# asonnino/hotstuff

Measured on NVIDIA H100. Metric: Ed25519 verifies/s, higher is better.
Workload: dtype u32

## Files before the change

hotstuff_b200/csrc/hs_engine.cu:

```cuda
#include <cuda_runtime.h>
#include <pthread.h>
#include <algorithm>
#include <array>
#include <atomic>
#include <chrono>
#include <condition_variable>
#include <cstdint>
#include <cstdio>
#include <cstdlib>
#include <cstring>
#include <deque>
#include <type_traits>
#include <initializer_list>
#include <list>
#include <memory>
#include <mutex>
#include <new>
#include <optional>
#include <random>
#include <string>
#include <string_view>
#include <system_error>
#include <thread>
#include <unordered_map>
#include <vector>

#include "../../include/hs_crypto.h"
#include "hs_args.h"
#include "hs_selftest_vectors.h"
#include "key_index.h"
#include "verify_core.cuh"

#define HS_THREADS 128
#define HS_FINISH_GROUP 16
#define HS_LEARN_MAX 8192u
#define HS_LEARN_PER_CALL 1024u
#define HS_CACHE_RESET_MIN_CALLS 64u

struct in_layout {
  const uint8_t *sig;
  size_t sig_stride;
  const uint8_t *pk;
  size_t pk_stride;
  const uint32_t *vidx;
  const uint8_t *msg;
  size_t msg_stride;
  const uint32_t *midx;
  const uint64_t *off;
  uint64_t fixed_len;
  int aos128;
};

__device__ __forceinline__ void load32(uint32_t (&w)[8], const uint8_t *p) {
  const uint32_t *s = reinterpret_cast<const uint32_t *>(p);
#pragma unroll
  for (int i = 0; i < 8; i++) w[i] = __ldg(s + i);
}
__device__ __forceinline__ void unpack8(uint32_t (&w)[8], uint4 lo, uint4 hi) {
  w[0] = lo.x; w[1] = lo.y; w[2] = lo.z; w[3] = lo.w;
  w[4] = hi.x; w[5] = hi.y; w[6] = hi.z; w[7] = hi.w;
}
__device__ __forceinline__ void store_digest32(uint32_t *dst, const uint32_t *h) {
  uint4 *d = reinterpret_cast<uint4 *>(dst);
  d[0] = make_uint4(h[0], h[1], h[2], h[3]);
  d[1] = make_uint4(h[4], h[5], h[6], h[7]);
}

template <class I, class Row>
__device__ __forceinline__ void warp_stage_rows128(uint4 (&q)[8], I n, I warp_first, Row row, uint4 *smem_warp, int lane) {
#pragma unroll
  for (int j = 0; j < 8; j++) {
    const int c = j * 32 + lane;
    const int rec = c >> 3, part = c & 7;
    const uint4 *src = row(rec);
    uint4 v = make_uint4(0, 0, 0, 0);
    if (warp_first + rec < n) v = __ldg(src + part);
    smem_warp[rec * 8 + (part ^ (rec & 7))] = v;
  }
  __syncwarp();
#pragma unroll
  for (int part = 0; part < 8; part++) q[part] = smem_warp[lane * 8 + (part ^ (lane & 7))];
}
__device__ __forceinline__ void warp_load_rec128(uint32_t (&sig_r)[8], uint32_t (&sig_s)[8], uint32_t (&pk)[8], uint32_t (&msg)[8],
                                                 const uint8_t *__restrict__ recs, size_t n, size_t warp_first, uint4 *smem_warp) {
  uint4 q[8];
  warp_stage_rows128(q, n, warp_first, [&](int r) { return reinterpret_cast<const uint4 *>(recs + (warp_first + r) * 128); }, smem_warp,
                     threadIdx.x & 31);
  __syncwarp();
  unpack8(sig_r, q[0], q[1]);
  unpack8(sig_s, q[2], q[3]);
  unpack8(pk, q[4], q[5]);
  unpack8(msg, q[6], q[7]);
}

struct key_table {
  const uint32_t *slots;
  uint32_t mask;
  const uint8_t *pks;
  uint32_t n_keys;
};
template <bool BOUNDED>
__device__ __forceinline__ uint32_t key_probe(const key_table &T, const uint32_t (&k)[8], uint32_t &pos) {
  uint32_t h = key_hash(k) & T.mask;
  for (uint32_t probe = 0; probe <= T.mask; probe++) {
    uint32_t idx = __ldg(T.slots + h);
    if (idx == HS_NO_KEY) break;
    if (!BOUNDED || idx < T.n_keys) {
      const uint32_t *cand = reinterpret_cast<const uint32_t *>(T.pks + (size_t)idx * 32);
      uint32_t diff = 0;
#pragma unroll
      for (int j = 0; j < 8; j++) diff |= __ldg(cand + j) ^ k[j];
      if (diff == 0) {
        pos = h;
        return idx;
      }
    }
    h = (h + 1) & T.mask;
  }
  return HS_NO_KEY;
}
__global__ void __launch_bounds__(256) k_key_lookup(in_layout L, size_t n, key_table T, uint32_t *__restrict__ out_vidx,
                                                    uint32_t *__restrict__ miss_list, uint32_t *__restrict__ miss_count) {
  const size_t i = (size_t)blockIdx.x * 256 + threadIdx.x;
  if (i >= n) return;
  uint32_t k[8];
  load32(k, L.pk + i * L.pk_stride);
  uint32_t pos;
  const uint32_t found = key_probe<false>(T, k, pos);
  out_vidx[i] = found;
  if (found == HS_NO_KEY) miss_list[atomicAdd(miss_count, 1u)] = (uint32_t)i;
}

__global__ void __launch_bounds__(256) k_gather_keys(in_layout L, size_t n, const uint32_t *__restrict__ miss_list,
                                                     const uint32_t *__restrict__ miss_count, uint32_t max_keys, uint8_t *__restrict__ out_keys,
                                                     uint32_t *__restrict__ out_n) {
  const size_t t = (size_t)blockIdx.x * 256 + threadIdx.x;
  const size_t avail = miss_count ? (size_t)*miss_count : n;
  const size_t take = avail < max_keys ? avail : max_keys;
  if (t == 0) *out_n = (uint32_t)take;
  if (t >= take) return;
  const size_t i = miss_count ? miss_list[t] : t;
  uint32_t k[8];
  load32(k, L.pk + i * L.pk_stride);
  uint32_t *dst = reinterpret_cast<uint32_t *>(out_keys + t * 32);
#pragma unroll
  for (int j = 0; j < 8; j++) dst[j] = k[j];
}

struct main_out {
  fe *xyz;
  uint8_t *meta;
  int side_pass;
};
struct committee_tables {
  const uint8_t *pks;
  const uint8_t *key_flags;
  uint32_t n_keys;
  const ge_niels *atables;
  size_t table_entries;
};

template <bool COMMITTEE>
#ifndef HS_MAIN_MINBLOCKS
#define HS_MAIN_MINBLOCKS 4
#endif
#ifndef HS_GENERIC_MINBLOCKS
#define HS_GENERIC_MINBLOCKS 3
#endif
__global__ void __launch_bounds__(HS_THREADS, COMMITTEE ? HS_MAIN_MINBLOCKS : HS_GENERIC_MINBLOCKS) k_verify_main(in_layout L, size_t n_arg, const uint32_t *__restrict__ n_ptr,
                                                             const uint32_t *__restrict__ index_list, const ge_niels *__restrict__ btable,
                                                             committee_tables C, main_out O, const comb_params cp) {
  __shared__ __align__(16) unsigned char smem_raw[HS_MAX_DIGITS * HS_THREADS * 4];
  static_assert(sizeof(smem_raw) >= (HS_THREADS / 32) * 256 * sizeof(uint4), "staging does not fit");
  uint4(*stage)[256] = reinterpret_cast<uint4(*)[256]>(smem_raw);
  int32_t *digits = reinterpret_cast<int32_t *>(smem_raw) + threadIdx.x;
  const size_t n = n_ptr ? (size_t)*n_ptr : n_arg;
  for (size_t base = (size_t)blockIdx.x * blockDim.x; base < n; base += (size_t)gridDim.x * blockDim.x) {
  const size_t t = base + threadIdx.x;
  const size_t warp_first = t & ~(size_t)31;
  const bool active = t < n;
  size_t i = active ? t : n - 1;
  uint32_t R[8], S[8], A[8], h[16];
  uint32_t v = 0;
  bool have_key = true;
  if (L.aos128 && !index_list) {
    uint32_t M[8];
    __syncthreads();
    warp_load_rec128(R, S, A, M, L.sig, n, warp_first, stage[threadIdx.x >> 5]);
    __syncthreads();
    if (COMMITTEE) {
      v = __ldg(L.vidx + i);
      have_key = v < C.n_keys;
      if (!have_key) v = 0;
      load32(A, C.pks + (size_t)v * 32);
    }
    sha512_ram32(h, R, A, M);
  } else {
    if (index_list) i = index_list[i];
    load32(R, L.sig + i * L.sig_stride);
    load32(S, L.sig + i * L.sig_stride + 32);
    if (COMMITTEE) {
      v = __ldg(L.vidx + i);
      have_key = v < C.n_keys;
      if (!have_key) v = 0;
      load32(A, C.pks + (size_t)v * 32);
    } else {
      load32(A, L.pk + i * L.pk_stride);
    }
    const uint8_t *m = L.off ? L.msg + L.off[i] : L.msg + (size_t)(L.midx ? __ldg(L.midx + i) : i) * L.msg_stride;
    const uint64_t len = L.off ? (L.off[i + 1] - L.off[i]) : L.fixed_len;
    if (len == 32 && ((reinterpret_cast<uintptr_t>(m) & 3u) == 0)) {
      uint32_t M[8];
      load32(M, m);
      sha512_ram32(h, R, A, M);
    } else {
      uint64_t pre[8];
#pragma unroll
      for (int j = 0; j < 4; j++) {
        pre[j] = be64_from_le32(R[2 * j], R[2 * j + 1]);
        pre[4 + j] = be64_from_le32(A[2 * j], A[2 * j + 1]);
      }
      sha512_prefix_msg(h, pre, 8, m, len);
    }
  }
  ge_ext acc;
  uint32_t meta;
  if (COMMITTEE) {
    meta = verify_committee_main(acc, R, S, h, btable, C.atables + (size_t)v * C.table_entries, have_key ? C.key_flags[v] : 0u, digits,
                                 HS_THREADS, cp);
    if (!have_key) {
      if (O.side_pass) continue;
      meta = 0;
    }
  } else {
    ge_cached tab[9];
    meta = verify_generic_main(acc, R, S, A, h, btable, tab, digits, HS_THREADS, cp);
  }
  if (!active) continue;
  if (!(meta & HS_META_PARSE_OK)) {
    fe_set0(acc.X);
    fe_set1(acc.Y);
    fe_set1(acc.Z);
  }
  uint4 *dst = reinterpret_cast<uint4 *>(O.xyz + i * 3);
  dst[0] = make_uint4(acc.X.v[0], acc.X.v[1], acc.X.v[2], acc.X.v[3]);
  dst[1] = make_uint4(acc.X.v[4], acc.X.v[5], acc.X.v[6], acc.X.v[7]);
  dst[2] = make_uint4(acc.Y.v[0], acc.Y.v[1], acc.Y.v[2], acc.Y.v[3]);
  dst[3] = make_uint4(acc.Y.v[4], acc.Y.v[5], acc.Y.v[6], acc.Y.v[7]);
  dst[4] = make_uint4(acc.Z.v[0], acc.Z.v[1], acc.Z.v[2], acc.Z.v[3]);
  dst[5] = make_uint4(acc.Z.v[4], acc.Z.v[5], acc.Z.v[6], acc.Z.v[7]);
  O.meta[i] = (uint8_t)meta;
  }
}

struct small_rec {
  uint8_t sig[64];
  uint8_t msg[32];
  uint32_t vidx;
  uint32_t req;
  uint32_t req_n;
  uint32_t pad[5];
};
static_assert(sizeof(small_rec) == 128, "small_rec is 128 bytes");
#define HS_SMALL_MAX 64
__device__ __forceinline__ void fe_shfl_down(fe &r, const fe &a, int delta) {
#pragma unroll
  for (int i = 0; i < 8; i++) r.v[i] = __shfl_down_sync(0xffffffffu, a.v[i], delta);
}

#define HS_SIG_WAYS 4
struct sig_entry {
  uint32_t w[32];
  uint32_t seq;
  uint32_t flags;
  uint32_t pad[2];
};
static_assert(sizeof(sig_entry) == 144, "sig_entry is 144 bytes");
struct sig_bucket {
  sig_entry e[HS_SIG_WAYS];
  uint32_t rr;
  uint32_t pad[3];
};
#define HS_SIG_CTRS 4
struct sig_cache_dev {
  sig_bucket *b;
  const uint64_t *key;
  uint32_t bmask;
  uint32_t *ctr;
  uint32_t *hctr;
};
#define HS_SIG_HIT 0x100u

__device__ __forceinline__ uint32_t ld_acquire_gpu(const uint32_t *p) {
  uint32_t v;
  asm volatile("ld.acquire.gpu.global.u32 %0, [%1];" : "=r"(v) : "l"(p) : "memory");
  return v;
}
__device__ __forceinline__ uint32_t ld_relaxed_gpu(const uint32_t *p) {
  uint32_t v;
  asm volatile("ld.relaxed.gpu.global.u32 %0, [%1];" : "=r"(v) : "l"(p) : "memory");
  return v;
}
__device__ __forceinline__ void st_relaxed_gpu(uint32_t *p, uint32_t v) {
  asm volatile("st.relaxed.gpu.global.u32 [%0], %1;" ::"l"(p), "r"(v) : "memory");
}
__device__ __forceinline__ uint64_t sig_mix(uint32_t w, uint64_t k) {
  uint64_t z = ((uint64_t)w << 32) ^ k;
  z = (z ^ (z >> 30)) * 0xbf58476d1ce4e5b9ull;
  z = (z ^ (z >> 27)) * 0x94d049bb133111ebull;
  return z ^ (z >> 31);
}
__device__ __forceinline__ uint32_t sig_bucket_of(const sig_cache_dev &sc, uint64_t h) { return (uint32_t)(h >> 32) & sc.bmask; }
__device__ __forceinline__ uint32_t pick8(const uint32_t (&a)[8], int i) {
  uint32_t r = a[0];
#pragma unroll
  for (int j = 1; j < 8; j++)
    if (i == j) r = a[j];
  return r;
}
__device__ __forceinline__ uint32_t sig_probe_warp(const sig_cache_dev &sc, uint32_t w, int lane, uint32_t &bucket) {
  uint64_t h = sig_mix(w, __ldg(sc.key + lane));
#pragma unroll
  for (int d = 16; d; d >>= 1) h += __shfl_xor_sync(0xffffffffu, h, d);
  bucket = sig_bucket_of(sc, h);
  const sig_entry *x = sc.b[bucket].e;
  uint32_t s0[HS_SIG_WAYS], m[HS_SIG_WAYS], f[HS_SIG_WAYS];
#pragma unroll
  for (int e = 0; e < HS_SIG_WAYS; e++) s0[e] = ld_acquire_gpu(&x[e].seq);
#pragma unroll
  for (int e = 0; e < HS_SIG_WAYS; e++) {
    m[e] = ld_relaxed_gpu(x[e].w + lane);
    f[e] = ld_relaxed_gpu(&x[e].flags);
  }
  __threadfence();
#pragma unroll
  for (int e = 0; e < HS_SIG_WAYS; e++) {
    const uint32_t s1 = ld_relaxed_gpu(&x[e].seq), s_lane0 = __shfl_sync(0xffffffffu, s0[e], 0), fl = __shfl_sync(0xffffffffu, f[e], 0);
    const bool ok = s0[e] != 0 && !(s0[e] & 1u) && s1 == s0[e] && s0[e] == s_lane0 && m[e] == w;
    if (__all_sync(0xffffffffu, ok)) return fl | HS_SIG_HIT;
  }
  return 0;
}
template <class W>
__device__ __forceinline__ uint32_t sig_probe_thread(const sig_cache_dev &sc, W word, uint32_t &bucket) {
  uint64_t h = 0;
#pragma unroll
  for (int j = 0; j < 32; j++) h += sig_mix(word(j), __ldg(sc.key + j));
  bucket = sig_bucket_of(sc, h);
  const sig_entry *x = sc.b[bucket].e;
#pragma unroll 1
  for (int e = 0; e < HS_SIG_WAYS; e++) {
    const uint32_t s0 = ld_acquire_gpu(&x[e].seq);
    if (!s0 || (s0 & 1u) || ld_relaxed_gpu(x[e].w) != word(0)) continue;
    bool eq = true;
#pragma unroll
    for (int j = 1; j < 32; j++) eq &= ld_relaxed_gpu(x[e].w + j) == word(j);
    const uint32_t fl = ld_relaxed_gpu(&x[e].flags);
    __threadfence();
    if (eq && ld_relaxed_gpu(&x[e].seq) == s0) return fl | HS_SIG_HIT;
  }
  return 0;
}
template <class W>
__device__ __forceinline__ uint32_t sig_insert(const sig_cache_dev &sc, uint32_t bucket, W word, uint32_t flags) {
// ... 1364 lines not shown
    cp.na = sc_ndigits_rt(w);
    sc_bias_rt(cp.bias_a, w);
  } else {
    cp.wb = w;
    cp.nb = sc_ndigits_rt(w);
    sc_bias_rt(cp.bias_b, w);
  }
}

static int audit_fence(hs_ctx *c, cudaStream_t stream) {
  c->key_gen++;
  c->map_gen++;
  if (c->audit.done) HS_CUDA(c, cudaStreamWaitEvent(stream, c->audit.done, 0));
  return HS_OK;
}
static void cache_release(hs_ctx *c) {
  c->key_gen++;
  c->map_gen++;
  c->keys = {};
  c->n_keys = 0;
  c->h_pks.clear();
  c->h_index = {};
  c->h_key_live.clear();
  c->stage = {};
  c->key_capacity = 0;
}
static int cache_allocate(hs_ctx *c, cudaStream_t stream) {
  size_t free_b = 0, total_b = 0;
  HS_CUDA(c, cudaMemGetInfo(&free_b, &total_b));
  size_t lim = free_b / 2;
  if (c->table_budget && c->table_budget < lim) lim = c->table_budget;
  int wa = 8;
  for (int w : {14, 12, 10, 8}) {
    if (c->wa_forced && w != c->wa_forced && w != 8) continue;
    wa = w;
    if (c->cache_cap * comb_table_entries(w) * sizeof(ge_niels) <= lim) break;
  }
  if (c->cache_cap * comb_table_entries(wa) * sizeof(ge_niels) > lim || sc_ndigits_rt(wa) + c->cp.nb > HS_MAX_DIGITS) {
    c->cache_enabled = false;
    return HS_OK;
  }
  set_window(c->cp, true, wa);
  c->a_table_entries = comb_table_entries(wa);
  HS_CUDA(c, make_key_store(c->keys, c->cache_cap, key_index::capacity_for(c->cache_cap), wa, stream));
  c->key_gen++;
  c->map_gen++;
  c->h_index.reset(c->cache_cap);
  c->h_pks.clear();
  return HS_OK;
}
static int learn_process(hs_ctx *c, cudaStream_t stream) {
  if (!c->learn_pending) return HS_OK;
  if (cudaEventQuery(c->learn.ev) != cudaSuccess) return HS_OK;
  c->learn_pending = false;
  c->calls_since_reset++;
  if (!c->cache_enabled || c->explicit_committee) return HS_OK;
  if (c->cache_full) {
    if (c->learn_records >= 64 && (size_t)*c->learn.h_miss_total * 2 > c->learn_records && c->calls_since_reset >= HS_CACHE_RESET_MIN_CALLS) {
      c->calls_since_reset = 0;
      HS_TRY(audit_fence(c, stream));
      c->n_keys = 0;
      c->h_pks.clear();
      c->h_index.clear();
      HS_CUDA(c, cudaMemsetAsync(c->keys.slots, 0xff, c->h_index.slots.size() * 4, stream));
      c->cache_full = false;
    }
    return HS_OK;
  }
  const uint32_t got = *c->learn.h_n < HS_LEARN_MAX ? *c->learn.h_n : HS_LEARN_MAX;
  if (got == 0) return HS_OK;
  if (!c->keys.atables) {
    HS_TRY(cache_allocate(c, stream));
    if (!c->cache_enabled) return HS_OK;
  }
  const size_t old_n = c->n_keys;
  size_t n_new = 0;
  for (uint32_t t = 0; t < got && old_n + n_new < c->cache_cap && n_new < HS_LEARN_PER_CALL; t++) {
    const uint8_t *key = c->learn.h_keys + 32 * (size_t)t;
    c->h_pks.insert(c->h_pks.end(), key, key + 32);
    if (c->h_index.insert_absent(c->h_pks.data(), (uint32_t)(old_n + n_new))) n_new++;
    else c->h_pks.resize(32 * (old_n + n_new));
  }
  if (n_new == 0) return HS_OK;
  HS_TRY(audit_fence(c, stream));
  HS_CUDA(c, cudaMemcpyAsync(c->keys.pks + old_n * 32, c->h_pks.data() + old_n * 32, n_new * 32, cudaMemcpyHostToDevice, stream));
  HS_CUDA(c, cudaMemcpyAsync(c->keys.slots, c->h_index.slots.data(), c->h_index.slots.size() * 4, cudaMemcpyHostToDevice, stream));
  HS_TRY(launch_build(c, c->keys.pks + old_n * 32, nullptr, n_new, 1, c->cp.wa, c->cp.na, c->keys.atables + old_n * c->a_table_entries,
                      c->keys.key_flags + old_n, stream));
  HS_CUDA(c, cudaEventRecord(c->learn.ev_tables, stream));
  c->n_keys = old_n + n_new;
  if (c->n_keys >= c->cache_cap) c->cache_full = true;
  return HS_OK;
}
static int learn_collect(hs_ctx *c, const in_layout &L, size_t n, bool have_lookup, cudaStream_t stream) {
  if (!c->cache_enabled || c->explicit_committee || c->learn_pending || !L.pk) return HS_OK;
  if (!c->learn.keys) {
    learn_bufs B;
    HS_CUDA(c, alloc(B.keys, (size_t)HS_LEARN_MAX * 32));
    HS_CUDA(c, alloc(B.n, 4));
    HS_CUDA(c, alloc(B.h_keys, (size_t)HS_LEARN_MAX * 32));
    HS_CUDA(c, alloc(B.h_n, 4));
    HS_CUDA(c, alloc(B.h_miss_total, 4));
    HS_CUDA(c, create(B.ev));
    HS_CUDA(c, create(B.ev_tables));
    c->learn = std::move(B);
  }
  learn_bufs &B = c->learn;
  c->learn_records = n;
  if (c->cache_full) {
    if (!have_lookup) return HS_OK;
    HS_CUDA(c, cudaMemcpyAsync(B.h_miss_total, c->d_miss_count, 4, cudaMemcpyDeviceToHost, stream));
    HS_CUDA(c, cudaEventRecord(B.ev, stream));
    c->learn_pending = true;
    return HS_OK;
  }
  k_gather_keys<<<blocks_for(HS_LEARN_MAX, 256), 256, 0, stream>>>(L, n, have_lookup ? (const uint32_t *)c->miss.p.get() : nullptr,
                                                                     have_lookup ? c->d_miss_count.get() : nullptr, HS_LEARN_MAX, B.keys, B.n);
  c->launches++;
  HS_CUDA(c, cudaGetLastError());
  HS_CUDA(c, cudaMemcpyAsync(B.h_n, B.n, 4, cudaMemcpyDeviceToHost, stream));
  HS_CUDA(c, cudaMemcpyAsync(B.h_keys, B.keys, (size_t)HS_LEARN_MAX * 32, cudaMemcpyDeviceToHost, stream));
  HS_CUDA(c, cudaEventRecord(B.ev, stream));
  c->learn_pending = true;
  return HS_OK;
}

struct pass_scratch {
  fe *xyz;
  uint8_t *meta;
  uint32_t *vidx, *miss, *miss_count;
  cudaStream_t side;
  cudaEvent_t ev_side[2];
  const event_h *prof;
};
struct pass_tables {
  committee_tables C;
  key_table T;
  comb_params cp;
};
static pass_tables store_tables(const key_store &S, const key_index &index, size_t n_keys, size_t entries, const comb_params &cp) {
  return pass_tables{{S.pks, S.key_flags, (uint32_t)n_keys, S.atables, entries}, {S.slots, index.mask, S.pks, (uint32_t)n_keys}, cp};
}
static pass_tables ctx_tables(const hs_ctx *c) { return store_tables(c->keys, c->h_index, c->n_keys, c->a_table_entries, c->cp); }
struct share_pass {
  sig_cache_dev sc;
  uint32_t *list;
  uint8_t *fl;
  uint32_t *h_ctr;
};
static int wait_key_cache_build(hs_ctx *c, cudaStream_t stream) {
  if (c->learn.ev_tables && !c->explicit_committee) HS_CUDA(c, cudaStreamWaitEvent(stream, c->learn.ev_tables, 0));
  return HS_OK;
}
template <class AfterLookup>
static int launch_main(hs_ctx *c, in_layout &L, size_t n, bool committee, bool indexed, const pass_tables &K, const pass_scratch &S,
                       cudaStream_t stream, AfterLookup after_lookup, const share_pass *sh = nullptr) {
  main_out O{S.xyz, S.meta, 0};
  const committee_tables &C = K.C;
  if (committee) {
    if (!indexed) {
      HS_CUDA(c, cudaMemsetAsync(S.miss_count, 0, 4, stream));
      k_key_lookup<<<blocks_for(n, 256), 256, 0, stream>>>(L, n, K.T, S.vidx, S.miss, S.miss_count);
      c->launches++;
      HS_CUDA(c, cudaGetLastError());
      L.vidx = S.vidx;
      O.side_pass = 1;
      HS_TRY(after_lookup(true));
      HS_CUDA(c, cudaEventRecord(S.ev_side[0], stream));
      HS_CUDA(c, cudaStreamWaitEvent(S.side, S.ev_side[0], 0));
      unsigned grid = blocks_for(n, 32);
      if (grid > c->n_sms * 8u) grid = c->n_sms * 8u;
      k_verify_main<false><<<grid, 32, 0, S.side>>>(L, 0, S.miss_count, S.miss, c->d_btable, C, O, K.cp);
      c->launches++;
      HS_CUDA(c, cudaGetLastError());
      HS_CUDA(c, cudaEventRecord(S.ev_side[1], S.side));
    }
    const uint32_t *n_ptr = nullptr, *list = nullptr;
    if (sh) {
      uint32_t *list_n = sh->sc.ctr + HS_SIG_CTRS;
      HS_CUDA(c, cudaMemsetAsync(sh->sc.ctr, 0, 4 * (HS_SIG_CTRS + 1), stream));
      k_sig_probe<<<blocks_for(n, 256), 256, 0, stream>>>(L, n, C, sh->sc, indexed ? 0 : 1, S.xyz, S.meta, sh->list, list_n);
      c->launches++;
      HS_CUDA(c, cudaGetLastError());
      n_ptr = list_n;
      list = sh->list;
    }
    if (S.prof) HS_CUDA(c, cudaEventRecord(S.prof[0], stream));
    k_verify_main<true><<<blocks_for(n), HS_THREADS, 0, stream>>>(L, n, n_ptr, list, c->d_btable, C, O, K.cp);
    if (S.prof) HS_CUDA(c, cudaEventRecord(S.prof[1], stream));
    c->launches++;
    HS_CUDA(c, cudaGetLastError());
    if (!indexed) HS_CUDA(c, cudaStreamWaitEvent(stream, S.ev_side[1], 0));
  } else {
    HS_TRY(after_lookup(false));
    k_verify_main<false><<<blocks_for(n), HS_THREADS, 0, stream>>>(L, n, nullptr, nullptr, c->d_btable, C, O, K.cp);
    c->launches++;
    HS_CUDA(c, cudaGetLastError());
  }
  return HS_OK;
}
static int launch_finish(hs_ctx *c, const in_layout &L, size_t n, const fe *xyz, const uint8_t *meta, uint32_t mode, const uint8_t *d_item_mode,
                         uint32_t *d_bitmap, const peer_route &P, int fin_group, cudaStream_t stream, const share_pass *sh = nullptr) {
  const size_t fin_threads = (n + fin_group - 1) / fin_group;
  if (sh && d_item_mode)
    k_verify_finish_modes_cached<<<blocks_for(fin_threads), HS_THREADS, 0, stream>>>(L, n, xyz, meta, d_item_mode, d_bitmap, P, fin_group, sh->fl);
  else if (sh)
    k_verify_finish_cached<<<blocks_for(fin_threads), HS_THREADS, 0, stream>>>(L, n, xyz, meta, mode, d_bitmap, P, fin_group, sh->fl);
  else if (d_item_mode)
    k_verify_finish_modes<<<blocks_for(fin_threads), HS_THREADS, 0, stream>>>(L, n, xyz, meta, d_item_mode, d_bitmap, P, fin_group);
  else
    k_verify_finish<<<blocks_for(fin_threads), HS_THREADS, 0, stream>>>(L, n, xyz, meta, mode, d_bitmap, P, fin_group);
  c->launches++;
  HS_CUDA(c, cudaGetLastError());
  return HS_OK;
}
static int launch_sig_fill(hs_ctx *c, const in_layout &L, size_t n, const committee_tables &C, const share_pass &sh, const uint8_t *meta,
                           uint32_t mode, const uint8_t *d_item_mode, cudaStream_t stream) {
  k_sig_fill<<<blocks_for(n, 256), 256, 0, stream>>>(L, n, C, sh.sc, meta, sh.fl, mode, d_item_mode);
  c->launches++;
  HS_CUDA(c, cudaGetLastError());
  HS_CUDA(c, cudaMemcpyAsync(sh.h_ctr, sh.sc.ctr, 4 * HS_SIG_CTRS, cudaMemcpyDeviceToHost, stream));
  return HS_OK;
}

static int run_verify(hs_ctx *c, in_layout L, size_t n, uint32_t mode, uint32_t *d_bitmap, cudaStream_t stream, bool indexed,
                      const uint8_t *d_item_mode = nullptr) {
  if (n == 0) {
    if (c->peer_armed) {
      c->peer_armed = false;
      k_peer_sync_only<<<1, HS_MAX_PEERS, 0, stream>>>(c->peers);
      c->launches++;
      HS_CUDA(c, cudaGetLastError());
    }
    return HS_OK;
  }
  if (indexed && !committee_registered(c)) return fail(c, HS_ERR_ARG, "committee-indexed verify without a registered committee");
  if (!indexed) HS_TRY(learn_process(c, stream));
  HS_TRY(wait_key_cache_build(c, stream));
  const bool defer = c->deferred && stream != c->stream;
  dev_buf &XYZ = (defer && c->flip) ? c->xyz2 : c->xyz, &META = (defer && c->flip) ? c->meta2 : c->meta;
  const int set = defer ? c->flip : 0;
  if (defer) {
    c->flip ^= 1;
    HS_CUDA(c, cudaStreamWaitEvent(stream, c->ev_tail[set], 0));
  }
  HS_TRY(ensure(c, XYZ, n * 3 * sizeof(fe)));
  HS_TRY(ensure(c, META, n));
  const bool committee = has_key_tables(c) && (indexed || L.pk);
  if (!committee && !L.pk) return fail(c, HS_ERR_ARG, "verify without keys");
  if (committee && !indexed) {
    HS_TRY(ensure(c, c->vidx, n * 4));
    HS_TRY(ensure(c, c->miss, n * 4));
  }
  const pass_scratch S{(fe *)XYZ.p.get(), (uint8_t *)META.p.get(), (uint32_t *)c->vidx.p.get(), (uint32_t *)c->miss.p.get(), c->d_miss_count, c->stream_side,
                       {c->ev_side[0], c->ev_side[1]}, c->profile_main ? c->ev_prof : nullptr};
  const bool share = c->share_sc.b && committee && stream == c->stream && !L.off && L.fixed_len == 32;
  share_pass SP{};
  if (share) {
    HS_TRY(ensure(c, c->share_list, n * 4));
    HS_TRY(ensure(c, c->share_fl, n));
    SP = share_pass{c->share_sc, (uint32_t *)c->share_list.p.get(), (uint8_t *)c->share_fl.p.get(), c->share_h.h};
  }
  HS_TRY(launch_main(c, L, n, committee, indexed, ctx_tables(c), S, stream,
                     [&](bool have_lookup) { return learn_collect(c, L, n, have_lookup, stream); }, share ? &SP : nullptr));
  const int fin_group = (defer || n >= (1u << 19)) ? 16 : (n >= (1u << 18) ? 8 : 4);
  peer_route P{};
  if (c->peer_armed) {
    P = c->peers;
    c->peer_armed = false;
  }
  cudaStream_t fin_stream = stream;
  if (defer) {
    HS_CUDA(c, cudaEventRecord(c->ev_main_done, stream));
    HS_CUDA(c, cudaStreamWaitEvent(c->stream_tail, c->ev_main_done, 0));
    fin_stream = c->stream_tail;
  }
  HS_TRY(launch_finish(c, L, n, (const fe *)XYZ.p.get(), (const uint8_t *)META.p.get(), mode, d_item_mode, d_bitmap, P, fin_group, fin_stream,
                       share ? &SP : nullptr));
  if (share) {
    HS_TRY(launch_sig_fill(c, L, n, ctx_tables(c).C, SP, (const uint8_t *)META.p.get(), mode, d_item_mode, stream));
    c->share_passes++;
  }
  if (defer) HS_CUDA(c, cudaEventRecord(c->ev_tail[set], c->stream_tail));
  if (fin_stream != c->stream) HS_CUDA(c, cudaEventRecord(c->ev_dev_pass, fin_stream));
  return HS_OK;
}

template <bool SIGC>
static cudaError_t launch_ring_verify_as(hs_ctx *c, const ring_bufs &r, uint32_t mask, uint32_t base, uint32_t n, bool bulk,
                                         const committee_tables &C, const comb_params &cp, const sig_cache_dev &sc, uint32_t seq, cudaStream_t s) {
  if (bulk)
    k_verify_bulk<SIGC><<<blocks_for(n, HS_BULK_THREADS), HS_BULK_THREADS, 0, s>>>(r.recs.d, base, mask, n, c->d_btable, C, cp, r.flags.d, r.counters,
                                                                                 r.done.d, seq, sc);
  else
    k_verify_small<SIGC><<<n, 64, 0, s>>>(r.recs.d, base, mask, c->d_btable, C, cp, r.flags.d, r.counters, r.done.d, seq, sc);
  c->launches++;
  return cudaGetLastError();
}
static cudaError_t launch_ring_verify(hs_ctx *c, const ring_bufs &r, uint32_t mask, uint32_t base, uint32_t n, bool bulk, const committee_tables &C,
                                      const comb_params &cp, const sig_cache_dev &sc, uint32_t seq, cudaStream_t s) {
  return sc.b ? launch_ring_verify_as<true>(c, r, mask, base, n, bulk, C, cp, sc, seq, s)
              : launch_ring_verify_as<false>(c, r, mask, base, n, bulk, C, cp, sc, seq, s);
}
static cudaError_t launch_queue_generic(hs_ctx *c, const ring_bufs &r, const uint8_t *pks, const uint32_t *slots, uint32_t mask, uint32_t base,
                                        uint32_t n, const comb_params &cp, uint32_t seq, cudaStream_t s) {
  k_queue_generic<<<blocks_for(n, HS_GEN_THREADS), HS_GEN_THREADS, 0, s>>>(r.recs.d, pks, slots, base, mask, n, c->d_btable, cp, r.flags.d,
                                                                         r.counters, r.done.d, seq);
  c->launches++;
  return cudaGetLastError();
}
static cudaError_t launch_queue_digests(hs_ctx *c, const ring_bufs &r, const qmsg_desc *list, uint32_t mask, uint32_t base, uint32_t n_desc,
                                        const uint8_t *arena, uint8_t *stage, uint32_t *digs, cudaStream_t s) {
  k_queue_digests<<<n_desc, HS_QDIG_THREADS, 0, s>>>(list, base, mask, arena, stage, digs, r.recs.d);
  c->launches++;
  return cudaGetLastError();
}
#define HS_QUEUE_EXPLAIN_SM_DIV 4
static cudaError_t launch_queue_explain(hs_ctx *c, const xq_desc *list, uint32_t n_desc, uint32_t n, uint8_t *mirror, uint8_t *arena,
                                        cudaStream_t s) {
  const unsigned grid = (unsigned)std::min<size_t>(blocks_for(n), std::max<size_t>(1, c->n_sms / HS_QUEUE_EXPLAIN_SM_DIV));
  k_queue_explain<<<grid, HS_THREADS, 0, s>>>(list, n_desc, n, mirror, arena);
  c->launches++;
  return cudaGetLastError();
}
static cudaError_t launch_sig_audit(hs_ctx *c, sig_bucket *b, uint32_t first, uint32_t n, unsigned long long *out, cudaStream_t s) {
  const unsigned grid = (unsigned)std::min<size_t>(blocks_for((size_t)n * HS_SIG_WAYS), std::max<size_t>(1, c->n_sms / HS_QUEUE_EXPLAIN_SM_DIV));
  k_sig_audit<<<grid, HS_THREADS, 0, s>>>(b, first, n, out);
  c->launches++;
  return cudaGetLastError();
}

static uint32_t host_key_lookup(const hs_ctx *c, const uint8_t *key) {
  return c->h_index.find(c->h_pks.data(), key, [c](uint32_t idx) { return idx < c->n_keys; });
}
static bool small_eligible(const hs_ctx *c, size_t n) { return c->small_enabled && n >= 1 && n <= HS_SMALL_MAX && has_key_tables(c); }
struct small_src {
  const uint8_t *sig, *msg;
  uint32_t vidx;
};
template <class Rec>
static bool small_stage(hs_ctx *c, size_t n, Rec rec) {
  bool all = true;
  for (size_t i = 0; i < n; i++) {
    const small_src s = rec(i);
    memcpy(c->small.recs.h[i].sig, s.sig, 64);
    memcpy(c->small.recs.h[i].msg, s.msg, 32);
    c->small.recs.h[i].vidx = s.vidx;
    all = all && s.vidx != HS_NO_KEY;
  }
  return all;
}
static int run_small(hs_ctx *c, size_t n, uint32_t mode, uint32_t *out_bitmap) {
  for (size_t i = 0; i < n; i++) {
    c->small.recs.h[i].req = 0;
    c->small.recs.h[i].req_n = (uint32_t)n;
  }
  const uint32_t seq = ++c->small_seq ? c->small_seq : ++c->small_seq;
  HS_TRY(wait_key_cache_build(c, c->stream));
  HS_CUDA(c, launch_ring_verify(c, c->small, HS_SMALL_MAX - 1, 0, (uint32_t)n, false, ctx_tables(c).C, c->cp, sig_cache_dev{}, seq, c->stream));
  volatile uint32_t *done = c->small.done.h;
  bool finished = false;
  for (uint64_t spin = 0; spin < (1ull << 34); spin++) {
    if (*done == seq) {
      finished = true;
      break;
    }
    if ((spin & 0xfff) == 0xfff) {
      cudaError_t q = cudaStreamQuery(c->stream);
      if (q != cudaSuccess && q != cudaErrorNotReady) return fail(c, HS_ERR_CUDA, "k_verify_small", q);
      if (q == cudaSuccess && *done != seq && spin > (1u << 20)) break;
    }
  }
  if (!finished) {
    HS_CUDA(c, cudaStreamSynchronize(c->stream));
    if (*done != seq) return fail(c, HS_ERR_CUDA, "k_verify_small did not complete");
  }
  for (size_t w = 0; w < (n + 31) / 32; w++) out_bitmap[w] = 0;
  const uint32_t want = mode_flag(mode);
  for (size_t i = 0; i < n; i++)
    if (((volatile uint8_t *)c->small.flags.h)[i] & want) out_bitmap[i >> 5] |= 1u << (i & 31);
  return HS_OK;
}

#define HS_QUEUE_DEFAULT_RECORDS 4096u
#define HS_QUEUE_MAX_RECORDS (1u << 20)
#define HS_QUEUE_MAX_INFLIGHT 2
#define HS_QUEUE_BULK_MIN 1002
static_assert(HS_QUEUE_BULK_MIN > HS_SMALL_MAX, "small requests never take the bulk path");
#define HS_QUEUE_ARENA_PER_RECORD 64u
struct queue_bits {
  uint32_t inl[(HS_SMALL_MAX + 31) / 32] = {0, 0};
  std::vector<uint32_t> big;
  void set(uint32_t n, const uint32_t *src_or_null) {
    const size_t w = (n + 31) / 32;
    uint32_t *d = inl;
    if (n > HS_SMALL_MAX) {
      big.assign(w, 0);
      d = big.data();
    } else {
      inl[0] = inl[1] = 0;
    }
    if (src_or_null) memcpy(d, src_or_null, 4 * w);
  }
  const uint32_t *data() const { return big.empty() ? inl : big.data(); }
};
struct ticket_sink {
  size_t ticket;
  hs_queue_cb *cb;
  void *user;
};
struct byte_ring {
  uint64_t cap = 0, head = 0, tail = 0;
  std::optional<uint64_t> take(uint64_t size) {
    uint64_t start = tail;
    if (off(start) + size > cap) start += cap - off(start);
    if (start + size - head > cap) {
      if (head != tail) return std::nullopt;
// ... 1056 lines not shown
  c->explicit_committee = true;
  c->h_pks.assign(pks, pks + N * 32);
  c->h_index = std::move(index);
  c->h_key_live.assign(N, 1);
  if (out_valid_bitmap) {
    for (size_t w = 0; w < (N + 31) / 32; w++) out_valid_bitmap[w] = 0;
    for (size_t i = 0; i < N; i++)
      if (fl[i] & 1) out_valid_bitmap[i >> 5] |= 1u << (i & 31);
  }
  return HS_OK;
}
int hs_committee_register(hs_ctx *c, const uint8_t *pks, size_t N, uint32_t *out_valid_bitmap) {
  if (!c || (N && !pks) || N >= HS_NO_KEY) return fail(c, HS_ERR_ARG, "hs_committee_register: bad argument");
  std::lock_guard<std::mutex> g(c->mu);
  return committee_register_locked(c, pks, N, out_valid_bitmap);
}

static int publish_hash(hs_ctx *c) {
  c->h_index.build(c->h_pks.data(), c->n_keys, [c](size_t i) { return !c->explicit_committee || c->h_key_live[i] == SLOT_LIVE; });
  HS_CUDA(c, cudaMemcpyAsync(c->keys.slots, c->h_index.slots.data(), c->h_index.slots.size() * 4, cudaMemcpyHostToDevice, c->stream));
  HS_CUDA(c, cudaStreamSynchronize(c->stream));
  return HS_OK;
}

struct slot_plan {
  std::vector<uint8_t> live, pks;
  std::vector<uint32_t> idx;
  std::vector<uint32_t> fresh;
  bool full = false;
};
static void plan_adds(const hs_ctx *c, const uint8_t *add_pks, size_t n_add, uint8_t mark, slot_plan &P) {
  P.live = c->h_key_live;
  P.pks = c->h_pks;
  key_index index = c->h_index;
  auto live = [&P](uint32_t idx) { return P.live[idx] != 0; };
  size_t next_free = 0;
  for (size_t i = 0; i < n_add; i++) {
    const uint8_t *key = add_pks + 32 * i;
    uint32_t idx = index.find(P.pks.data(), key, live);
    if (idx == HS_NO_KEY) {
      while (next_free < P.live.size() && P.live[next_free]) next_free++;
      if (next_free < P.live.size()) idx = (uint32_t)next_free;
      else if (P.live.size() < c->key_capacity) {
        idx = (uint32_t)P.live.size();
        P.live.push_back(0);
        P.pks.resize(P.live.size() * 32);
      } else {
        P.full = true;
        return;
      }
      memcpy(P.pks.data() + 32 * (size_t)idx, key, 32);
      P.live[idx] = mark;
      index.insert_absent(P.pks.data(), idx, live);
      P.fresh.push_back(idx);
    }
    P.idx.push_back(idx);
  }
}
static void stage_drop(hs_ctx *c) {
  for (uint32_t s : c->stage.fresh)
    if (s < c->h_key_live.size() && c->h_key_live[s] == SLOT_STAGED) c->h_key_live[s] = 0;
  if (c->explicit_committee && c->h_key_live.size() > c->n_keys) c->h_key_live.resize(c->n_keys);
  c->stage = {};
}

int hs_committee_update(hs_ctx *c, const uint8_t *add_pks, size_t n_add, const uint32_t *remove_idx, size_t n_remove, uint32_t *out_add_idx) {
  if (!c || (n_add && (!add_pks || !out_add_idx)) || (n_remove && !remove_idx)) return fail(c, HS_ERR_ARG, "hs_committee_update: bad argument");
  std::lock_guard<std::mutex> g(c->mu);
  if (!c->explicit_committee) return fail(c, HS_ERR_ARG, "hs_committee_update: no committee registered");
  HS_CUDA(c, cudaSetDevice(c->device));
  HS_CUDA(c, cudaDeviceSynchronize());
  for (size_t i = 0; i < n_remove; i++)
    if (remove_idx[i] >= c->n_keys) return fail(c, HS_ERR_ARG, "hs_committee_update: remove index out of range");
  stage_drop(c);
  c->key_gen++;
  c->map_gen++;
  for (size_t i = 0; i < n_remove; i++) {
    c->h_key_live[remove_idx[i]] = 0;
    HS_CUDA(c, cudaMemsetAsync(c->keys.key_flags + remove_idx[i], 0, 1, c->stream));
  }
  slot_plan P;
  plan_adds(c, add_pks, n_add, SLOT_LIVE, P);
  c->h_key_live = std::move(P.live);
  c->h_pks = std::move(P.pks);
  c->n_keys = c->h_key_live.size();
  std::copy(P.idx.begin(), P.idx.end(), out_add_idx);
  const size_t n_new = P.fresh.size();
  if (n_new) {
    for (uint32_t s : P.fresh)
      HS_CUDA(c, cudaMemcpyAsync(c->keys.pks + 32 * (size_t)s, c->h_pks.data() + 32 * (size_t)s, 32, cudaMemcpyHostToDevice, c->stream));
    h2d_stage st;
    const size_t s_slots = st.add(P.fresh.data(), 4 * n_new), s_flags = st.add(nullptr, n_new);
    HS_TRY(st.upload(c, c->in[0], c->stream));
    HS_TRY(launch_build(c, c->keys.pks, reinterpret_cast<const uint32_t *>(st.ptr(s_slots)), n_new, 1, c->cp.wa, c->cp.na, c->keys.atables,
                        st.ptr(s_flags), c->stream));
    for (size_t k = 0; k < n_new; k++)
      HS_CUDA(c, cudaMemcpyAsync(c->keys.key_flags + P.fresh[k], st.ptr(s_flags) + k, 1, cudaMemcpyDeviceToDevice, c->stream));
  }
  if (P.full) {
    HS_CUDA(c, cudaStreamSynchronize(c->stream));
    return fail(c, HS_ERR_NOMEM, "hs_committee_update: no free table slot (re-register the committee)");
  }
  HS_TRY(publish_hash(c));
  return HS_OK;
}
int hs_set_table_budget(hs_ctx *c, size_t bytes) {
  if (!c) return HS_ERR_ARG;
  std::lock_guard<std::mutex> g(c->mu);
  c->table_budget = bytes;
  return HS_OK;
}

int hs_verify_rec128_dev(hs_ctx *c, const void *d_recs, size_t n, uint32_t mode, void *d_bitmap, void *stream) {
  if (!c || (n && (!d_recs || !d_bitmap)) || mode > 1) return fail(c, HS_ERR_ARG, "hs_verify_rec128_dev: bad argument");
  HS_CUDA(c, cudaSetDevice(c->device));
  return run_verify(c, layout_rec128(d_recs), n, mode, (uint32_t *)d_bitmap, (cudaStream_t)stream, false);
}
int hs_verify_var_dev(hs_ctx *c, const void *d_sig, const void *d_pk, const void *d_msgs, const void *d_off, size_t n, uint32_t mode,
                      void *d_bitmap, void *stream) {
  if (!c || mode > 1 || (n && (!d_sig || !d_pk || !d_off || !d_bitmap))) return fail(c, HS_ERR_ARG, "hs_verify_var_dev: bad argument");
  HS_CUDA(c, cudaSetDevice(c->device));
  in_layout L{(const uint8_t *)d_sig, 64, (const uint8_t *)d_pk, 32, nullptr, (const uint8_t *)d_msgs, 0, nullptr, (const uint64_t *)d_off, 0, 0};
  return run_verify(c, L, n, mode, (uint32_t *)d_bitmap, (cudaStream_t)stream, false);
}
int hs_verify_committee_dev(hs_ctx *c, const void *d_vidx, const void *d_sig, const void *d_midx, const void *d_digests, size_t n,
                            uint32_t mode, void *d_bitmap, void *stream) {
  if (!c || mode > 1 || (n && (!d_vidx || !d_sig || !d_digests || !d_bitmap))) return fail(c, HS_ERR_ARG, "hs_verify_committee_dev: bad argument");
  HS_CUDA(c, cudaSetDevice(c->device));
  in_layout L{(const uint8_t *)d_sig, 64, nullptr, 0, (const uint32_t *)d_vidx, (const uint8_t *)d_digests, d_midx ? (size_t)32 : (size_t)0,
              (const uint32_t *)d_midx, nullptr, 32, 0};
  return run_verify(c, L, n, mode, (uint32_t *)d_bitmap, (cudaStream_t)stream, true);
}
int hs_digest32_dev(hs_ctx *c, const void *d_data, const void *d_off, size_t n, void *d_out, void *stream) {
  if (!c || (n && (!d_off || !d_out))) return fail(c, HS_ERR_ARG, "hs_digest32_dev: bad argument");
  if (n == 0) return HS_OK;
  HS_CUDA(c, cudaSetDevice(c->device));
  k_digest32<<<blocks_for(n), HS_THREADS, 0, (cudaStream_t)stream>>>((const uint8_t *)d_data, (const uint64_t *)d_off, 0, n, (uint32_t *)d_out);
  c->launches++;
  HS_CUDA(c, cudaGetLastError());
  return HS_OK;
}
int hs_digest32_fixed_dev(hs_ctx *c, const void *d_msgs, size_t msg_len, size_t n, void *d_out, void *stream) {
  if (!c || (n && (!d_msgs || !d_out || msg_len == 0))) return fail(c, HS_ERR_ARG, "hs_digest32_fixed_dev: bad argument");
  if (n == 0) return HS_OK;
  HS_CUDA(c, cudaSetDevice(c->device));
  return launch_digest_fixed(c, (const uint8_t *)d_msgs, msg_len, n, (uint32_t *)d_out, (cudaStream_t)stream);
}
int hs_verify_msgs_dev(hs_ctx *c, const void *d_sig, const void *d_pk, const void *d_vidx, const void *d_msgs, size_t msg_len, size_t n,
                       uint32_t mode, void *d_digests, void *d_bitmap, void *stream) {
  if (!c || mode > 1 || (n && (!d_sig || (!d_pk && !d_vidx) || !d_msgs || !d_digests || !d_bitmap)))
    return fail(c, HS_ERR_ARG, "hs_verify_msgs_dev: bad argument");
  if (n == 0) return HS_OK;
  HS_CUDA(c, cudaSetDevice(c->device));
  HS_TRY(launch_digest_fixed(c, (const uint8_t *)d_msgs, msg_len, n, (uint32_t *)d_digests, (cudaStream_t)stream));
  in_layout L{(const uint8_t *)d_sig, 64, (const uint8_t *)d_pk, 32, (const uint32_t *)d_vidx, (const uint8_t *)d_digests, 32, nullptr, nullptr, 32, 0};
  return run_verify(c, L, n, mode, (uint32_t *)d_bitmap, (cudaStream_t)stream, d_vidx != nullptr);
}

int hs_verify_qcs(hs_ctx *c, const uint8_t *preimages, size_t n_qc, const uint8_t *pk, const uint32_t *vidx, const uint8_t *sig,
                  const uint32_t *qc_idx, size_t n_votes, uint32_t *out_vote_bitmap, uint32_t *out_qc_bitmap) {
  if (!c || !out_qc_bitmap || (n_qc && !preimages) || (n_votes && (!sig || !qc_idx || (!pk && !vidx) || n_qc == 0)))
    return fail(c, HS_ERR_ARG, "hs_verify_qcs: bad argument");
  for (size_t i = 0; i < n_votes; i++)
    if (qc_idx[i] >= n_qc) return fail(c, HS_ERR_ARG, "hs_verify_qcs: qc_idx out of range");
  const size_t qc_words = (n_qc + 31) / 32, vote_words = (n_votes + 31) / 32;
  const std::vector<uint32_t> ones = bitmap_ones(n_qc);
  if (n_votes == 0) {
    std::copy(ones.begin(), ones.end(), out_qc_bitmap);
    return HS_OK;
  }
  std::lock_guard<std::mutex> g(c->mu);
  share_call sh(c);
  HS_CUDA(c, cudaSetDevice(c->device));
  h2d_stage S;
  const size_t s_pre = S.add(preimages, n_qc * 40), s_dig = S.add(nullptr, n_qc * 32), s_sig = S.add(sig, n_votes * 64),
               s_key = S.add(pk ? (const void *)pk : (const void *)vidx, n_votes * (pk ? 32 : 4)), s_qi = S.add(qc_idx, n_votes * 4);
  HS_TRY(ensure(c, c->out, (vote_words + qc_words) * 4));
  HS_TRY(S.upload(c, c->in[0], c->stream));
  uint32_t *d_votes = (uint32_t *)c->out.p.get(), *d_qc = d_votes + vote_words;
  const uint32_t *d_qi = (const uint32_t *)S.ptr(s_qi);
  HS_CUDA(c, cudaMemcpyAsync(d_qc, ones.data(), qc_words * 4, cudaMemcpyHostToDevice, c->stream));
  k_digest32<<<blocks_for(n_qc), HS_THREADS, 0, c->stream>>>(S.ptr(s_pre), nullptr, 40, n_qc, (uint32_t *)S.ptr(s_dig));
  c->launches++;
  HS_CUDA(c, cudaGetLastError());
  HS_TRY(hs_verify_qc_votes_dev(c, S.ptr(s_dig), pk ? S.ptr(s_key) : nullptr, pk ? nullptr : S.ptr(s_key), S.ptr(s_sig), d_qi, n_votes, d_votes,
                                c->stream));
  HS_TRY(launch_qc_and(c, d_votes, d_qi, n_votes, n_qc, d_qc, c->stream));
  return readback(c, {{out_vote_bitmap, d_votes, vote_words * 4}, {out_qc_bitmap, d_qc, qc_words * 4}});
}

int hs_verify_qc_votes_dev(hs_ctx *c, const void *d_qc_digests, const void *d_pk, const void *d_vidx, const void *d_sig, const void *d_qc_idx,
                           size_t n_votes, void *d_vote_bitmap, void *stream) {
  if (!c || (n_votes && (!d_qc_digests || (!d_pk && !d_vidx) || !d_sig || !d_qc_idx || !d_vote_bitmap)))
    return fail(c, HS_ERR_ARG, "hs_verify_qc_votes_dev: bad argument");
  HS_CUDA(c, cudaSetDevice(c->device));
  in_layout L{(const uint8_t *)d_sig, 64, (const uint8_t *)d_pk, 32, (const uint32_t *)d_vidx, (const uint8_t *)d_qc_digests, 32,
              (const uint32_t *)d_qc_idx, nullptr, 32, 0};
  return run_verify(c, L, n_votes, HS_MODE_BATCH_EQ, (uint32_t *)d_vote_bitmap, (cudaStream_t)stream, d_pk == nullptr);
}
int hs_qc_and_dev(hs_ctx *c, const void *d_vote_bitmap, const void *d_qc_idx, size_t n_votes, size_t n_qc, void *d_qc_bitmap, void *stream) {
  if (!c || !d_qc_bitmap || (n_votes && (!d_vote_bitmap || !d_qc_idx))) return fail(c, HS_ERR_ARG, "hs_qc_and_dev: bad argument");
  HS_CUDA(c, cudaSetDevice(c->device));
  cudaStream_t st = (c->deferred && (cudaStream_t)stream != c->stream) ? c->stream_tail : (cudaStream_t)stream;
  if (n_qc) k_bitmap_ones<<<blocks_for((n_qc + 31) / 32, 256), 256, 0, st>>>((uint32_t *)d_qc_bitmap, n_qc);
  c->launches += n_qc ? 1 : 0;
  HS_CUDA(c, cudaGetLastError());
  if (n_votes) HS_TRY(launch_qc_and(c, (const uint32_t *)d_vote_bitmap, (const uint32_t *)d_qc_idx, n_votes, n_qc, (uint32_t *)d_qc_bitmap, st));
  return HS_OK;
}

int hs_verify_groups_dev(hs_ctx *c, const void *d_pre, const void *d_off, size_t n_msgs, const void *d_sig, const void *d_pk, const void *d_vidx,
                         const void *d_msg_idx, const void *d_mode, size_t n_items, void *d_item_bitmap, void *stream) {
  if (!c || (n_items && (!d_pre || !d_off || !d_sig || (!d_pk && !d_vidx) || !d_msg_idx || !d_item_bitmap)))
    return fail(c, HS_ERR_ARG, "hs_verify_groups_dev: bad argument");
  if (n_items && n_msgs == 0) return fail(c, HS_ERR_ARG, "hs_verify_groups_dev: items without preimages");
  if (n_items && !d_pk && !committee_registered(c))
    return fail(c, HS_ERR_ARG, "hs_verify_groups_dev: committee-indexed items without a registered committee");
  HS_CUDA(c, cudaSetDevice(c->device));
  if (n_items == 0) return run_verify(c, in_layout{}, 0, HS_MODE_STRICT, nullptr, (cudaStream_t)stream, false);
  HS_TRY(ensure(c, c->group_digests, n_msgs * 32));
  uint8_t *dig = (uint8_t *)c->group_digests.p.get();
  HS_TRY(hs_digest32_dev(c, d_pre, d_off, n_msgs, dig, stream));
  in_layout L{(const uint8_t *)d_sig, 64, (const uint8_t *)d_pk, 32, (const uint32_t *)d_vidx, dig, 32, (const uint32_t *)d_msg_idx, nullptr, 32, 0};
  return run_verify(c, L, n_items, HS_MODE_STRICT, (uint32_t *)d_item_bitmap, (cudaStream_t)stream, d_pk == nullptr, (const uint8_t *)d_mode);
}

int hs_verify_tcs(hs_ctx *c, const uint64_t *tc_rounds, size_t n_tc, const uint8_t *pk, const uint32_t *vidx, const uint8_t *sig,
                  const uint64_t *high_qc_rounds, const uint32_t *tc_idx, size_t n_votes, uint32_t *out_vote_bitmap, uint32_t *out_tc_bitmap) {
  if (!c || !out_tc_bitmap || (n_tc && !tc_rounds) || (n_votes && (!sig || !high_qc_rounds || (!pk && !vidx) || n_tc == 0)) || (!tc_idx && n_votes && n_tc != n_votes))
    return fail(c, HS_ERR_ARG, "hs_verify_tcs: bad argument");
  if (tc_idx)
    for (size_t i = 0; i < n_votes; i++)
      if (tc_idx[i] >= n_tc) return fail(c, HS_ERR_ARG, "hs_verify_tcs: tc_idx out of range");
  const size_t tc_words = (n_tc + 31) / 32, vote_words = (n_votes + 31) / 32;
  const std::vector<uint32_t> ones = bitmap_ones(n_tc);
  if (n_votes == 0) {
    std::copy(ones.begin(), ones.end(), out_tc_bitmap);
    return HS_OK;
  }
  std::lock_guard<std::mutex> g(c->mu);
  share_call sh(c);
  HS_CUDA(c, cudaSetDevice(c->device));
  h2d_stage S;
  const size_t s_r = S.add(tc_rounds, n_tc * 8), s_hq = S.add(high_qc_rounds, n_votes * 8), s_dig = S.add(nullptr, n_votes * 32),
               s_sig = S.add(sig, n_votes * 64), s_key = S.add(pk ? (const void *)pk : (const void *)vidx, n_votes * (pk ? 32 : 4)),
               s_ti = S.add(tc_idx, n_votes * 4);
  HS_TRY(ensure(c, c->out, (vote_words + tc_words) * 4));
  HS_TRY(S.upload(c, c->in[0], c->stream));
  uint32_t *d_votes = (uint32_t *)c->out.p.get(), *d_tc = d_votes + vote_words;
  const uint32_t *d_ti = tc_idx ? (const uint32_t *)S.ptr(s_ti) : nullptr;
  if (tc_idx) HS_CUDA(c, cudaMemcpyAsync(d_tc, ones.data(), tc_words * 4, cudaMemcpyHostToDevice, c->stream));
  k_tc_digests<<<blocks_for(n_votes), HS_THREADS, 0, c->stream>>>((const uint64_t *)S.ptr(s_r), d_ti, (const uint64_t *)S.ptr(s_hq), n_votes, n_tc,
                                                                  (uint32_t *)S.ptr(s_dig));
  c->launches++;
  HS_CUDA(c, cudaGetLastError());
  in_layout L{S.ptr(s_sig), 64, pk ? S.ptr(s_key) : nullptr, 32, pk ? nullptr : (const uint32_t *)S.ptr(s_key), S.ptr(s_dig), 32, nullptr, nullptr, 32, 0};
  HS_TRY(run_verify(c, L, n_votes, HS_MODE_STRICT, d_votes, c->stream, pk == nullptr));
  if (tc_idx) HS_TRY(launch_qc_and(c, d_votes, d_ti, n_votes, n_tc, d_tc, c->stream));
  return readback(c, {{out_vote_bitmap, d_votes, vote_words * 4}, {out_tc_bitmap, tc_idx ? d_tc : d_votes, tc_words * 4}});
}

int hs_verify_groups(hs_ctx *c, const uint8_t *preimages, const uint64_t *pre_off, size_t n_msgs, const uint8_t *sig, const uint8_t *pk,
                     const uint32_t *vidx, const uint32_t *msg_idx, const uint32_t *group_idx, const uint8_t *mode, size_t n_items, size_t n_groups,
                     uint32_t *out_item_bitmap, uint32_t *out_group_bitmap) {
  if (!c) return HS_ERR_ARG;
  if (const char *why = hs_args::groups(preimages, pre_off, n_msgs, sig, pk, vidx, msg_idx, group_idx, mode, n_items, n_groups, out_group_bitmap))
    return fail_args(c, "hs_verify_groups", why);
  const size_t g_words = (n_groups + 31) / 32, i_words = (n_items + 31) / 32;
  const std::vector<uint32_t> ones = bitmap_ones(n_groups);
  if (n_items == 0) {
    std::copy(ones.begin(), ones.end(), out_group_bitmap);
    return HS_OK;
  }
  std::lock_guard<std::mutex> g(c->mu);
  share_call sh(c);
  HS_CUDA(c, cudaSetDevice(c->device));
  h2d_stage S;
  const size_t s_off = S.add(pre_off, (n_msgs + 1) * 8), s_pre = S.add(preimages, pre_off[n_msgs], 8), s_sig = S.add(sig, n_items * 64),
               s_key = S.add(pk ? (const void *)pk : (const void *)vidx, n_items * (pk ? 32 : 4)), s_mi = S.add(msg_idx, n_items * 4),
               s_gi = S.add(group_idx, n_items * 4), s_mo = S.add(mode, n_items);
  HS_TRY(ensure(c, c->out, (i_words + g_words) * 4));
  HS_TRY(S.upload(c, c->in[0], c->stream));
  uint32_t *d_items = (uint32_t *)c->out.p.get(), *d_groups = d_items + i_words;
  HS_CUDA(c, cudaMemcpyAsync(d_groups, ones.data(), g_words * 4, cudaMemcpyHostToDevice, c->stream));
  HS_TRY(hs_verify_groups_dev(c, S.ptr(s_pre), S.ptr(s_off), n_msgs, S.ptr(s_sig), pk ? S.ptr(s_key) : nullptr, pk ? nullptr : S.ptr(s_key),
                              S.ptr(s_mi), mode ? S.ptr(s_mo) : nullptr, n_items, d_items, c->stream));
  HS_TRY(launch_qc_and(c, d_items, (const uint32_t *)S.ptr(s_gi), n_items, n_groups, d_groups, c->stream));
  return readback(c, {{out_item_bitmap, d_items, i_words * 4}, {out_group_bitmap, d_groups, g_words * 4}});
}

int hs_keygen_batch_dev(hs_ctx *c, const void *d_seeds, size_t n, void *d_pks, void *stream) {
  if (!c || (n && (!d_seeds || !d_pks))) return fail(c, HS_ERR_ARG, "hs_keygen_batch_dev: bad argument");
  if (n == 0) return HS_OK;
  HS_CUDA(c, cudaSetDevice(c->device));
  k_keygen<<<blocks_for(n), HS_THREADS, 0, (cudaStream_t)stream>>>((const uint8_t *)d_seeds, n, c->d_btable, c->cp, (uint8_t *)d_pks);
  c->launches++;
  HS_CUDA(c, cudaGetLastError());
  return HS_OK;
}
int hs_sign_digests_dev(hs_ctx *c, const void *d_seeds, const void *d_pks, size_t n_keys, const void *d_key_idx, const void *d_digests, size_t n,
                        void *d_sig, void *stream) {
  if (!c || (n && (!d_seeds || !d_pks || !d_digests || !d_sig || n_keys == 0)) || (!d_key_idx && n > n_keys))
    return fail(c, HS_ERR_ARG, "hs_sign_digests_dev: bad argument");
  if (n == 0) return HS_OK;
  HS_CUDA(c, cudaSetDevice(c->device));
  k_sign_digests<<<blocks_for(n), HS_THREADS, 0, (cudaStream_t)stream>>>((const uint8_t *)d_seeds, (const uint8_t *)d_pks, (const uint32_t *)d_key_idx,
                                                                          (const uint8_t *)d_digests, n, n_keys, c->d_btable, c->cp, (uint8_t *)d_sig);
  c->launches++;
  HS_CUDA(c, cudaGetLastError());
// ... 1925 lines not shown
```

Measured before the change: 259.5 million.

## Overlap message digest with committee key-miss verify pass on side stream

In hs_verify_msgs_dev, the message digest kernel no longer runs before everything else. It now launches after the key lookup, so the miss-path verify on the side stream can run alongside it. The miss pass does not wait for precomputed digests; it hashes the raw message inline, using a new in_layout mode flag. The miss pass launch also moves from 32-thread to 64-thread blocks with a lower grid cap. This adds redundant hashing for missed keys and a special-case branch inside the main verify kernel.

```diff
diff --git a/hotstuff_b200/csrc/hs_engine.cu b/hotstuff_b200/csrc/hs_engine.cu
--- a/hotstuff_b200/csrc/hs_engine.cu
+++ b/hotstuff_b200/csrc/hs_engine.cu
@@ -50,6 +50,7 @@
   uint64_t fixed_len;
   int aos128;
 };
+#define HS_IN_MSG_DIGEST 2
 
 __device__ __forceinline__ void load32(uint32_t (&w)[8], const uint8_t *p) {
   const uint32_t *s = reinterpret_cast<const uint32_t *>(p);
@@ -209,7 +210,14 @@
     }
     const uint8_t *m = L.off ? L.msg + L.off[i] : L.msg + (size_t)(L.midx ? __ldg(L.midx + i) : i) * L.msg_stride;
     const uint64_t len = L.off ? (L.off[i + 1] - L.off[i]) : L.fixed_len;
-    if (len == 32 && ((reinterpret_cast<uintptr_t>(m) & 3u) == 0)) {
+    if (!COMMITTEE && L.aos128 == HS_IN_MSG_DIGEST) {
+      uint32_t d[16], M[8];
+      const uint64_t none[8] = {0, 0, 0, 0, 0, 0, 0, 0};
+      sha512_prefix_msg(d, none, 0, m, len);
+#pragma unroll
+      for (int j = 0; j < 8; j++) M[j] = d[j];
+      sha512_ram32(h, R, A, M);
+    } else if (len == 32 && ((reinterpret_cast<uintptr_t>(m) & 3u) == 0)) {
       uint32_t M[8];
       load32(M, m);
       sha512_ram32(h, R, A, M);
@@ -1880,9 +1888,25 @@
   if (c->learn.ev_tables && !c->explicit_committee) HS_CUDA(c, cudaStreamWaitEvent(stream, c->learn.ev_tables, 0));
   return HS_OK;
 }
+struct msgs_digest {
+  const uint8_t *msgs;
+  size_t msg_len;
+  uint32_t *digests;
+};
+static int launch_digest_fixed(hs_ctx *c, const uint8_t *d_msgs, size_t msg_len, size_t n, uint32_t *d_out, cudaStream_t stream);
+
+static int launch_miss_pass(hs_ctx *c, const in_layout &L, size_t n, const pass_tables &K, const pass_scratch &S, const main_out &O) {
+  unsigned grid = blocks_for(n, 64);
+  if (grid > c->n_sms * 4u) grid = c->n_sms * 4u;
+  k_verify_main<false><<<grid, 64, 0, S.side>>>(L, 0, S.miss_count, S.miss, c->d_btable, K.C, O, K.cp);
+  c->launches++;
+  HS_CUDA(c, cudaGetLastError());
+  return HS_OK;
+}
+
 template <class AfterLookup>
 static int launch_main(hs_ctx *c, in_layout &L, size_t n, bool committee, bool indexed, const pass_tables &K, const pass_scratch &S,
-                       cudaStream_t stream, AfterLookup after_lookup, const share_pass *sh = nullptr) {
+                       cudaStream_t stream, AfterLookup after_lookup, const share_pass *sh = nullptr, const msgs_digest *md = nullptr) {
   main_out O{S.xyz, S.meta, 0};
   const committee_tables &C = K.C;
   if (committee) {
@@ -1896,13 +1920,18 @@
       HS_TRY(after_lookup(true));
       HS_CUDA(c, cudaEventRecord(S.ev_side[0], stream));
       HS_CUDA(c, cudaStreamWaitEvent(S.side, S.ev_side[0], 0));
-      unsigned grid = blocks_for(n, 32);
-      if (grid > c->n_sms * 8u) grid = c->n_sms * 8u;
-      k_verify_main<false><<<grid, 32, 0, S.side>>>(L, 0, S.miss_count, S.miss, c->d_btable, C, O, K.cp);
-      c->launches++;
-      HS_CUDA(c, cudaGetLastError());
+      if (md) {
+        in_layout Ls = L;
+        Ls.msg = md->msgs;
+        Ls.msg_stride = Ls.fixed_len = md->msg_len;
+        Ls.aos128 = HS_IN_MSG_DIGEST;
+        HS_TRY(launch_miss_pass(c, Ls, n, K, S, O));
+      } else {
+        HS_TRY(launch_miss_pass(c, L, n, K, S, O));
+      }
       HS_CUDA(c, cudaEventRecord(S.ev_side[1], S.side));
     }
+    if (md) HS_TRY(launch_digest_fixed(c, md->msgs, md->msg_len, n, md->digests, stream));
     const uint32_t *n_ptr = nullptr, *list = nullptr;
     if (sh) {
       uint32_t *list_n = sh->sc.ctr + HS_SIG_CTRS;
@@ -1920,6 +1949,7 @@
     HS_CUDA(c, cudaGetLastError());
     if (!indexed) HS_CUDA(c, cudaStreamWaitEvent(stream, S.ev_side[1], 0));
   } else {
+    if (md) HS_TRY(launch_digest_fixed(c, md->msgs, md->msg_len, n, md->digests, stream));
     HS_TRY(after_lookup(false));
     k_verify_main<false><<<blocks_for(n), HS_THREADS, 0, stream>>>(L, n, nullptr, nullptr, c->d_btable, C, O, K.cp);
     c->launches++;
@@ -1952,7 +1982,7 @@
 }
 
 static int run_verify(hs_ctx *c, in_layout L, size_t n, uint32_t mode, uint32_t *d_bitmap, cudaStream_t stream, bool indexed,
-                      const uint8_t *d_item_mode = nullptr) {
+                      const uint8_t *d_item_mode = nullptr, const msgs_digest *md = nullptr) {
   if (n == 0) {
     if (c->peer_armed) {
       c->peer_armed = false;
@@ -1990,7 +2020,7 @@
     SP = share_pass{c->share_sc, (uint32_t *)c->share_list.p.get(), (uint8_t *)c->share_fl.p.get(), c->share_h.h};
   }
   HS_TRY(launch_main(c, L, n, committee, indexed, ctx_tables(c), S, stream,
-                     [&](bool have_lookup) { return learn_collect(c, L, n, have_lookup, stream); }, share ? &SP : nullptr));
+                     [&](bool have_lookup) { return learn_collect(c, L, n, have_lookup, stream); }, share ? &SP : nullptr, md));
   const int fin_group = (defer || n >= (1u << 19)) ? 16 : (n >= (1u << 18) ? 8 : 4);
   peer_route P{};
   if (c->peer_armed) {
@@ -3353,9 +3383,9 @@
     return fail(c, HS_ERR_ARG, "hs_verify_msgs_dev: bad argument");
   if (n == 0) return HS_OK;
   HS_CUDA(c, cudaSetDevice(c->device));
-  HS_TRY(launch_digest_fixed(c, (const uint8_t *)d_msgs, msg_len, n, (uint32_t *)d_digests, (cudaStream_t)stream));
   in_layout L{(const uint8_t *)d_sig, 64, (const uint8_t *)d_pk, 32, (const uint32_t *)d_vidx, (const uint8_t *)d_digests, 32, nullptr, nullptr, 32, 0};
-  return run_verify(c, L, n, mode, (uint32_t *)d_bitmap, (cudaStream_t)stream, d_vidx != nullptr);
+  const msgs_digest md{(const uint8_t *)d_msgs, msg_len, (uint32_t *)d_digests};
+  return run_verify(c, L, n, mode, (uint32_t *)d_bitmap, (cudaStream_t)stream, d_vidx != nullptr, nullptr, &md);
 }
 
 int hs_verify_qcs(hs_ctx *c, const uint8_t *preimages, size_t n_qc, const uint8_t *pk, const uint32_t *vidx, const uint8_t *sig,
```

New measurement: 266.2 million, median of 6. 1.03x the previous value.
